# seung-lab/chunkflow

Measured on AMD Instinct MI355X. Metric: output_voxels_per_sec, higher is better.
Workload: dtype f32; 1 GPU; config2-512cube-rsunet-affinity; batch_size=12, engine=rsunet

## Files before the change

### chunkflow_amd/csrc/updown.hip

```cpp
#include <hip/hip_runtime.h>
#include <hip/hip_bf16.h>

#include "cfx_internal.h"

namespace {

typedef __hip_bfloat16 cfx_bf16;

template <typename T>
__device__ __forceinline__ float ldf(const T* p);
template <>
__device__ __forceinline__ float ldf<float>(const float* p) { return *p; }
template <>
__device__ __forceinline__ float ldf<cfx_bf16>(const cfx_bf16* p) {
    return __bfloat162float(*p);
}
__device__ __forceinline__ float cvf(float v) { return v; }
__device__ __forceinline__ float cvf(cfx_bf16 v) {
    return __bfloat162float(v);
}

template <typename T>
struct vec4;
template <>
struct vec4<float> {
    typedef float type __attribute__((ext_vector_type(4)));
    static __device__ __forceinline__ float get(type v, int i) {
        return v[i];
    }
};
template <>
struct vec4<cfx_bf16> {
    typedef unsigned short type __attribute__((ext_vector_type(4)));
    static __device__ __forceinline__ float get(type v, int i) {
        return __bfloat162float(
            __hip_bfloat16(__hip_bfloat16_raw{(unsigned short)v[i]}));
    }
};
template <typename T>
__device__ __forceinline__ void stf(T* p, float v);
template <>
__device__ __forceinline__ void stf<float>(float* p, float v) { *p = v; }
template <>
__device__ __forceinline__ void stf<cfx_bf16>(cfx_bf16* p, float v) {
    *p = __float2bfloat16(v);
}

template <typename T>
__device__ __forceinline__ void stage_rows(
    float* s_in, const T* in, const long long* row_off, int rows, int xn,
    int xvalid, int C, int CPAD, int tid, int nthreads) {
    const int total = rows * xn * C;
    for (int idx = tid; idx < total; idx += nthreads) {
        const int c = idx % C;
// ... 17 lines not shown
    float* s_in = smem + C * K * 4;
    const int CPAD = C | 1;
    const int tid = threadIdx.x;
    const int kslot = tid & 31;
    const int pslot = tid >> 5;

    for (int idx = tid; idx < C * K * 4; idx += 256) {
        const int q = idx & 3;
        const int k = (idx >> 2) % K;
        const int c = (idx >> 2) / K;
        s_w[(c * K + k) * 4 + q] = ldf(&wgt[(q * C + c) * K + k]);
    }

    const int nz = blockIdx.z;
    const int y = blockIdx.y;
    const int x0 = blockIdx.x * XI;
    const int xvalid = min(XI, W - x0);
    long long row_off[1] = {((((long long)nz * H) + y) * W + x0) * C};
    stage_rows(s_in, in, row_off, 1, XI, xvalid, C, CPAD, tid, 256);
    __syncthreads();

    const long long out_base =
        ((((long long)nz * 2 * H) + 2 * y) * 2 * W) * K;

    for (int k = kslot; k < K; k += 32) {
        const float bj = bias ? bias[k] : 0.f;
        float acc[PX][4];
#pragma unroll
        for (int p = 0; p < PX; ++p)
#pragma unroll
            for (int q = 0; q < 4; ++q) acc[p][q] = bj;
        for (int c = 0; c < C; ++c) {
            const float4 w4 =
                *reinterpret_cast<const float4*>(&s_w[(c * K + k) * 4]);
#pragma unroll
            for (int p = 0; p < PX; ++p) {
                const float v = s_in[(pslot + p * 8) * CPAD + c];
                acc[p][0] += v * w4.x;
                acc[p][1] += v * w4.y;
                acc[p][2] += v * w4.z;
                acc[p][3] += v * w4.w;
            }
        }
#pragma unroll
        for (int p = 0; p < PX; ++p) {
            const int xi = x0 + pslot + p * 8;
            if (xi >= W) continue;
            T* op = out + out_base + (long long)2 * xi * K + k;
            stf(op, acc[p][0]);
            stf(op + K, acc[p][1]);
            stf(op + (long long)2 * W * K, acc[p][2]);
            stf(op + (long long)2 * W * K + K, acc[p][3]);
        }
    }
}

template <typename T, int XO>
__global__ __launch_bounds__(256, 2) void k_downconv2(
    const T* __restrict__ in, const T* __restrict__ wgt,
    const float* __restrict__ bias, T* __restrict__ out, int N, int D,
    int H, int W, int C, int K) {
    constexpr int PX = XO / 8;
    extern __shared__ float smem[];
    float* s_w = smem;
    float* s_in = smem + C * K * 4;
    const int CPAD = C | 1;
    const int tid = threadIdx.x;
    const int kslot = tid & 31;
    const int pslot = tid >> 5;
    const int HO = H >> 1, WO = W >> 1;

    for (int idx = tid; idx < C * K * 4; idx += 256) {
        const int q = idx & 3;
        const int k = (idx >> 2) % K;
        const int c = (idx >> 2) / K;
        s_w[(c * K + k) * 4 + q] = ldf(&wgt[(q * C + c) * K + k]);
    }

    const int nz = blockIdx.z;
    const int y = blockIdx.y;
    const int x0 = blockIdx.x * XO;
    const int xvalid = min(2 * XO, W - 2 * x0);
    long long row_off[2] = {
        ((((long long)nz * H) + 2 * y) * W + 2 * x0) * C,
        ((((long long)nz * H) + 2 * y + 1) * W + 2 * x0) * C};
    stage_rows(s_in, in, row_off, 2, 2 * XO, xvalid, C, CPAD, tid, 256);
    __syncthreads();

    const long long out_row = (((long long)nz * HO) + y) * WO * K;

    for (int k = kslot; k < K; k += 32) {
        const float bj = bias ? bias[k] : 0.f;
        float acc[PX];
#pragma unroll
        for (int p = 0; p < PX; ++p) acc[p] = bj;
        for (int c = 0; c < C; ++c) {
            const float4 w4 =
                *reinterpret_cast<const float4*>(&s_w[(c * K + k) * 4]);
#pragma unroll
            for (int p = 0; p < PX; ++p) {
                const int xl = 2 * (pslot + p * 8);
                acc[p] += s_in[xl * CPAD + c] * w4.x;
                acc[p] += s_in[(xl + 1) * CPAD + c] * w4.y;
                acc[p] += s_in[(2 * XO + xl) * CPAD + c] * w4.z;
                acc[p] += s_in[(2 * XO + xl + 1) * CPAD + c] * w4.w;
            }
// ... 225 lines not shown
    const int q = tid - yl * (CO_S / 4);
    const int y = y0 + yl;
    const int gx = x0 + q * 4;
    if (y >= H || gx >= W) return;
    float o[4][3];
#pragma unroll
    for (int e = 0; e < 4; ++e)
#pragma unroll
        for (int k = 0; k < 3; ++k) o[e][k] = bias ? bias[k] : 0.f;
#pragma unroll
    for (int j = 0; j < 15; ++j) {
        const int dx = j / 3, k = j % 3;
        const float* pr = &s_p[(yl * 16 + j) * CO_PS + q * 4];
        const co_f32x4 lo = *reinterpret_cast<const co_f32x4*>(pr);
        const co_f32x4 hi = *reinterpret_cast<const co_f32x4*>(pr + 4);
        const float p8[8] = {lo[0], lo[1], lo[2], lo[3],
                             hi[0], hi[1], hi[2], hi[3]};
#pragma unroll
        for (int e = 0; e < 4; ++e) o[e][k] += p8[e + dx];
    }
    T* op = out + ((plane + y) * W + gx) * 3LL;
    if (vec_ok) {
        if (sizeof(T) == 2) {
            typedef unsigned co_u32x2 __attribute__((ext_vector_type(2)));
            unsigned short h[12];
#pragma unroll
            for (int i = 0; i < 12; ++i) h[i] = bf16_bits(o[i / 3][i % 3]);
#pragma unroll
            for (int i = 0; i < 3; ++i) {
                co_u32x2 u;
                u.x = h[4 * i] | ((unsigned)h[4 * i + 1] << 16);
                u.y = h[4 * i + 2] | ((unsigned)h[4 * i + 3] << 16);
                reinterpret_cast<co_u32x2*>(op)[i] = u;
            }
        } else {
#pragma unroll
            for (int i = 0; i < 3; ++i) {
                co_f32x4 f;
#pragma unroll
                for (int m = 0; m < 4; ++m)
                    f[m] = o[(4 * i + m) / 3][(4 * i + m) % 3];
                reinterpret_cast<co_f32x4*>(op)[i] = f;
            }
        }
    } else {
#pragma unroll
        for (int e = 0; e < 4; ++e)
            if (gx + e < W)
#pragma unroll
                for (int k = 0; k < 3; ++k) stf(&op[e * 3 + k], o[e][k]);
    }
}

}

extern "C" int cfx_conv155_out(cfx_ctx* ctx, const void* in,
                               const float* wfrag, const float* bias,
                               void* out, int N, int D, int H, int W,
                               int C, int K, int is_bf16) {
    if (C != 28 || K != 3) {
        g_err = "cfx_conv155_out: only C == 28, K == 3 instantiated";
        return -1;
    }
    if ((long long)N * D > 65535) {
        g_err = "cfx_conv155_out: N * D <= 65535 supported";
        return -1;
    }
    hipEvent_t e0;
    if (prof_begin(ctx, &e0)) return -1;
    dim3 grid((W + CO_S - 1) / CO_S, (H + CO_R - 1) / CO_R,
              (unsigned)(N * D));
    const int vec_ok = W % 4 == 0 && ((size_t)out & 15) == 0;
    if (is_bf16)
        hipLaunchKernelGGL((k_conv155_out_mfma<cfx_bf16>), grid, dim3(256),
                           0, ctx->stream, (const cfx_bf16*)in, wfrag, bias,
                           (cfx_bf16*)out, H, W, vec_ok);
    else
        hipLaunchKernelGGL((k_conv155_out_mfma<float>), grid, dim3(256), 0,
                           ctx->stream, (const float*)in, wfrag, bias,
                           (float*)out, H, W, vec_ok);
    CFX_CHECK(hipGetLastError());
    double flops = 2.0 * 25.0 * C * K * (double)N * D * H * W;
    if (prof_end(ctx, e0, CFX_K_CONV_STREAM, flops)) return -1;
    return 0;
}

extern "C" int cfx_conv155_c1(cfx_ctx* ctx, const void* in, const void* wgt,
                              const float* bias, void* out, int N, int D,
                              int H, int W, int K, int is_bf16) {
    if (K > 32) {
        g_err = "cfx_conv155_c1: K <= 32 supported";
        return -1;
    }
    constexpr int XI = 256;
    dim3 grid((W + XI - 1) / XI, H, (unsigned)(N * D));
    hipEvent_t e0;
    if (prof_begin(ctx, &e0)) return -1;
    if (is_bf16 && K == 28)
        hipLaunchKernelGGL((k_conv155_c1<cfx_bf16, XI, 28>), grid,
                           dim3(XI), 0, ctx->stream, (const cfx_bf16*)in,
                           (const cfx_bf16*)wgt, bias, (cfx_bf16*)out, N,
                           D, H, W, K);
    else if (is_bf16)
        hipLaunchKernelGGL((k_conv155_c1<cfx_bf16, XI, 0>), grid,
                           dim3(XI), 0, ctx->stream, (const cfx_bf16*)in,
                           (const cfx_bf16*)wgt, bias, (cfx_bf16*)out, N,
                           D, H, W, K);
    else if (K == 28)
        hipLaunchKernelGGL((k_conv155_c1<float, XI, 28>), grid, dim3(XI),
                           0, ctx->stream, (const float*)in,
                           (const float*)wgt, bias, (float*)out, N, D, H,
                           W, K);
    else
        hipLaunchKernelGGL((k_conv155_c1<float, XI, 0>), grid, dim3(XI),
                           0, ctx->stream, (const float*)in,
                           (const float*)wgt, bias, (float*)out, N, D, H,
                           W, K);
    CFX_CHECK(hipGetLastError());
    double flops = 2.0 * 25.0 * K * (double)N * D * H * W;
    if (prof_end(ctx, e0, CFX_K_CONV_STREAM, flops)) return -1;
    return 0;
}

extern "C" int cfx_upconv_2x2(cfx_ctx* ctx, const void* in, const void* wgt,
                              const float* bias, void* out, int N, int D,
                              int H, int W, int C, int K, int is_bf16) {
    if (K > 64 || C > 64) {
        g_err = "cfx_upconv_2x2: C, K <= 64 supported";
        return -1;
    }
    constexpr int XI = 64;
    dim3 grid((W + XI - 1) / XI, H, (unsigned)(N * D));
    const size_t shmem =
        ((size_t)C * K * 4 + (size_t)XI * (C | 1)) * sizeof(float);
    hipEvent_t e0;
    if (prof_begin(ctx, &e0)) return -1;
    if (is_bf16)
        hipLaunchKernelGGL((k_upconv2<cfx_bf16, XI>), grid, dim3(256),
                           shmem, ctx->stream, (const cfx_bf16*)in,
                           (const cfx_bf16*)wgt, bias, (cfx_bf16*)out, N, D,
                           H, W, C, K);
    else
        hipLaunchKernelGGL((k_upconv2<float, XI>), grid, dim3(256), shmem,
                           ctx->stream, (const float*)in, (const float*)wgt,
                           bias, (float*)out, N, D, H, W, C, K);
    CFX_CHECK(hipGetLastError());
    double flops = 2.0 * 4.0 * C * K * (double)N * D * H * W;
    if (prof_end(ctx, e0, CFX_K_CONV_STREAM, flops)) return -1;
    return 0;
}

extern "C" int cfx_downconv_2x2(cfx_ctx* ctx, const void* in,
                                const void* wgt, const float* bias,
                                void* out, int N, int D, int H, int W,
                                int C, int K, int is_bf16) {
    if (K > 64 || C > 64) {
        g_err = "cfx_downconv_2x2: C, K <= 64 supported";
        return -1;
    }
    if ((H | W) & 1) {
        g_err = "cfx_downconv_2x2: H, W must be even";
        return -1;
    }
    constexpr int XO = 64;
    dim3 grid((W / 2 + XO - 1) / XO, H / 2, (unsigned)(N * D));
    const size_t shmem =
        ((size_t)C * K * 4 + (size_t)2 * 2 * XO * (C | 1)) * sizeof(float);
    hipEvent_t e0;
    if (prof_begin(ctx, &e0)) return -1;
    if (is_bf16)
        hipLaunchKernelGGL((k_downconv2<cfx_bf16, XO>), grid, dim3(256),
                           shmem, ctx->stream, (const cfx_bf16*)in,
                           (const cfx_bf16*)wgt, bias, (cfx_bf16*)out, N, D,
                           H, W, C, K);
    else
        hipLaunchKernelGGL((k_downconv2<float, XO>), grid, dim3(256), shmem,
                           ctx->stream, (const float*)in, (const float*)wgt,
                           bias, (float*)out, N, D, H, W, C, K);
    CFX_CHECK(hipGetLastError());
    double flops = 2.0 * 4.0 * C * K * (double)N * D * (H / 2) * (W / 2);
    if (prof_end(ctx, e0, CFX_K_CONV_STREAM, flops)) return -1;
    return 0;
}
```

### chunkflow_amd/engines/pytorch.py

```python
import os

import torch

from .base import EngineBase
from ..model_loader import load_source


class PyTorchEngine(EngineBase):
    pre_masked = False

    def __init__(self, convnet_model, convnet_weight_path, **kw):
        super().__init__(convnet_model, convnet_weight_path, **kw)
        net_source = load_source(convnet_model)
        if hasattr(net_source, 'load_model'):
            self.model = net_source.load_model(convnet_weight_path)
        else:
            self.model = net_source.InstantiatedModel
            if convnet_weight_path is not None:
                chkpt = torch.load(convnet_weight_path,
                                   map_location='cpu')
                state_dict = chkpt.get('state_dict', chkpt) \
                    if isinstance(chkpt, dict) else chkpt
                self.model.load_state_dict(state_dict)
        self.model = self.model.to(self.device)
        self.model.eval()
        if self.dtype == 'bfloat16':
            self.model = self.model.to(torch.bfloat16)
        self.channels_last = (str(self.device).startswith('cuda') and
                              os.environ.get('CFX_CHANNELS_LAST', '1') != '0')
        if self.channels_last:
            self.model = self.model.to(memory_format=torch.channels_last_3d)
            if os.environ.get('CFX_FASTCONV', '1') != '0':
                idx = int(str(self.device).split(':')[-1])                     if ':' in str(self.device) else 0
                from ..fastconv import (accelerate_conv_in,
                                        accelerate_updown)
                bf = self.dtype == 'bfloat16'
                if bf:
                    from ..fastconv import maybe_accelerate_bf16
                    self.fastconv_count = maybe_accelerate_bf16(
                        self.model, idx)
                else:
                    from ..fastconv import maybe_accelerate
                    self.fastconv_count = maybe_accelerate(self.model, idx)
                self.fastconv_count += accelerate_updown(
                    self.model, idx, bf16=bf)
                self.fastconv_count += accelerate_conv_in(
                    self.model, idx, bf16=bf)
                from ..fastconv import accelerate_conv_out
                self.fastconv_count += accelerate_conv_out(
                    self.model, idx, bf16=bf)
        torch.backends.cudnn.benchmark = True
        self.pre_process = getattr(net_source, 'pre_process', None)
        self.post_process = getattr(net_source, 'post_process', None)

    @torch.no_grad()
    def __call__(self, batch):
        x = batch
        if self.pre_process is not None:
            x = self.pre_process(x)
        if self.dtype == 'bfloat16':
            x = x.to(torch.bfloat16)
        if self.channels_last:
            x = x.contiguous(memory_format=torch.channels_last_3d)
        out = self.model(x)
        if self.post_process is not None:
            out = self.post_process(out)
        if out.dtype != torch.float32:
            out = out.to(torch.float32)
        out = self._crop_output_patch(out)
        return out.contiguous()
```

### chunkflow_amd/fastconv.py

```python
import os

import torch
import torch.nn as nn

_CTX = {}


def get_cfx(device_index: int = 0):
    if device_index not in _CTX:
        from .hip import CfxContext
        ctx = CfxContext(device_index)
        ctx.adopt_torch_stream()
        _CTX[device_index] = ctx
    return _CTX[device_index]


ELIGIBLE_WIDTHS = (28, 36)
ZRING_WIDTHS = (28, 36)


def _eligible(m: nn.Module) -> bool:
    return (isinstance(m, nn.Conv3d)
            and m.kernel_size == (3, 3, 3)
            and m.stride == (1, 1, 1)
# ... 9 lines not shown
    def __init__(self, conv: nn.Conv3d, device_index: int = 0):
        super().__init__()
        self.C = conv.in_channels
        self.K = conv.out_channels
        self.device_index = device_index
        w = conv.weight.detach()
        wtap = w.permute(2, 3, 4, 1, 0).reshape(27, self.C, self.K)
        self.register_buffer('wtap', wtap.contiguous().float())
        if conv.bias is not None:
            self.register_buffer('bias', conv.bias.detach().float())
        else:
            self.bias = None

    def _run(self, x, residual=None, elu=False):
        x = x.contiguous(memory_format=torch.channels_last_3d)
        n, c, d, h, w = x.shape
        out = torch.empty((n, self.K, d, h, w), dtype=torch.float32,
                          device=x.device,
                          memory_format=torch.channels_last_3d)
        get_cfx(self.device_index).conv3_ndhwc(
            x.data_ptr(), self.wtap.data_ptr(),
            self.bias.data_ptr() if self.bias is not None else None,
            residual.data_ptr() if residual is not None else None,
            out.data_ptr(), n, d, h, w, self.C, self.K, do_elu=elu,
            zring=self.C in ZRING_WIDTHS)
        return out

    def forward(self, x):
        assert x.dtype == torch.float32, 'fastconv is the f32 path'
        return self._run(x)


class CfxResBlock(nn.Module):

    def __init__(self, block: nn.Module, device_index: int = 0):
        super().__init__()
        self.c1 = CfxConv3d(block.conv1, device_index)
        self.c2 = CfxConv3d(block.conv2, device_index)

    def forward(self, x):
        x = x.contiguous(memory_format=torch.channels_last_3d)
        h = self.c1._run(x, elu=True)
        return self.c2._run(h, residual=x, elu=True)


def _resblock_like(m: nn.Module) -> bool:
    return (hasattr(m, 'conv1') and hasattr(m, 'conv2')
            and isinstance(getattr(m, 'act', None), nn.ELU)
            and getattr(m.act, 'alpha', None) == 1.0
            and not isinstance(m, (CfxConv3d, CfxResBlock))
            and _eligible(m.conv1) and _eligible(m.conv2))


@torch.no_grad()
def _fusion_matches(block: nn.Module, fused: 'CfxResBlock') -> bool:
    C = fused.c1.C
    x = torch.randn(1, C, 4, 18, 22, device=fused.c1.wtap.device)         .contiguous(memory_format=torch.channels_last_3d)
    want = block.to(x.device)(x)
    got = fused(x)
    return bool(torch.allclose(got, want, rtol=1e-4, atol=1e-4))


def maybe_accelerate(model: nn.Module, device_index: int = 0) -> int:
    count = 0
    dev = f'cuda:{device_index}'
    fused_out = set()
    for parent in list(model.modules()):
        if id(parent) in fused_out:
            continue
        for name, child in list(parent.named_children()):
            if _resblock_like(child):
                fused = CfxResBlock(child, device_index).to(dev)
                if _fusion_matches(child, fused):
                    setattr(parent, name, fused)
                    fused_out.add(id(child))
                    count += 1
                    continue
                for cn in ('conv1', 'conv2'):
                    setattr(child, cn,
                            CfxConv3d(getattr(child, cn),
                                      device_index).to(dev))
                    count += 1
            elif _eligible(child):
                setattr(parent, name,
                        CfxConv3d(child, device_index).to(dev))
                count += 1
    return count


BF16_WIDTHS = tuple(
    int(w) for w in os.environ.get('CFX_BF16_WIDTHS', '28,36').split(',')
    if w)


class CfxConv3dBF16(nn.Module):

    def __init__(self, conv: nn.Conv3d, device_index: int = 0):
        super().__init__()
        self.C = conv.in_channels
        self.K = conv.out_channels
        self.device_index = device_index
        w = conv.weight.detach().float()
        if self.C <= 32:
            pack = torch.zeros(27, 32, 32)
        else:
            pack = torch.zeros(27, 64, 48)
        pack[:, :self.K, :self.C] = w.permute(2, 3, 4, 0, 1) \
            .reshape(27, self.K, self.C)
        self.register_buffer('wpack', pack.to(torch.bfloat16).contiguous())
        if conv.bias is not None:
            self.register_buffer('bias', conv.bias.detach().float())
        else:
            self.bias = None

    def _run(self, x, residual=None, elu=False):
        assert x.dtype == torch.bfloat16
        x = x.contiguous(memory_format=torch.channels_last_3d)
        n, c, d, h, w = x.shape
        out = torch.empty((n, self.K, d, h, w), dtype=torch.bfloat16,
                          device=x.device,
                          memory_format=torch.channels_last_3d)
        get_cfx(self.device_index).conv3_ndhwc_bf16(
            x.data_ptr(), self.wpack.data_ptr(),
            self.bias.data_ptr() if self.bias is not None else None,
            residual.data_ptr() if residual is not None else None,
            out.data_ptr(), n, d, h, w, self.C, self.K, do_elu=elu)
        return out

    def forward(self, x):
        return self._run(x)


class CfxResBlockBF16(nn.Module):
    def __init__(self, block: nn.Module, device_index: int = 0):
# ... 27 lines not shown

    @torch.no_grad()
    def matches(block, fused):
        x = torch.randn(1, fused.c1.C, 4, 18, 22, device=dev) \
            .to(torch.bfloat16) \
            .contiguous(memory_format=torch.channels_last_3d)
        want = block.to(dev)(x)
        got = fused(x)
        return bool(torch.allclose(got.float(), want.float(), rtol=0.05,
                                   atol=0.05))

    fused_out = set()
    for parent in list(model.modules()):
        if id(parent) in fused_out:
            continue
        for name, child in list(parent.named_children()):
            if rb(child):
                fused = CfxResBlockBF16(child, device_index).to(dev)
                if matches(child, fused):
                    setattr(parent, name, fused)
                    fused_out.add(id(child))
                    count += 1
                    continue
                for cn in ('conv1', 'conv2'):
                    setattr(child, cn,
                            CfxConv3dBF16(getattr(child, cn),
                                          device_index).to(dev))
                    count += 1
            elif elig(child):
                setattr(parent, name,
                        CfxConv3dBF16(child, device_index).to(dev))
                count += 1
    return count


class CfxUpConv3d(nn.Module):

    def __init__(self, conv: nn.ConvTranspose3d, device_index: int = 0,
                 bf16: bool = False):
        super().__init__()
        self.C = conv.in_channels
        self.K = conv.out_channels
        self.device_index = device_index
        self.bf16 = bf16
        w = conv.weight.detach().float()
        pack = w[:, :, 0].permute(2, 3, 0, 1).reshape(4, self.C, self.K)
        dt = torch.bfloat16 if bf16 else torch.float32
        self.register_buffer('wpack', pack.to(dt).contiguous())
        if conv.bias is not None:
            self.register_buffer('bias', conv.bias.detach().float())
        else:
            self.bias = None

    def forward(self, x):
        x = x.contiguous(memory_format=torch.channels_last_3d)
        n, c, d, h, w = x.shape
        dt = torch.bfloat16 if self.bf16 else torch.float32
        assert x.dtype == dt
        out = torch.empty((n, self.K, d, 2 * h, 2 * w), dtype=dt,
                          device=x.device,
                          memory_format=torch.channels_last_3d)
        get_cfx(self.device_index).upconv_2x2(
            x.data_ptr(), self.wpack.data_ptr(),
            self.bias.data_ptr() if self.bias is not None else None,
            out.data_ptr(), n, d, h, w, self.C, self.K, bf16=self.bf16)
        return out


class CfxDownConv3d(nn.Module):

    def __init__(self, conv: nn.Conv3d, device_index: int = 0,
                 bf16: bool = False):
        super().__init__()
        self.C = conv.in_channels
        self.K = conv.out_channels
        self.device_index = device_index
        self.bf16 = bf16
        w = conv.weight.detach().float()
        pack = w[:, :, 0].permute(2, 3, 1, 0).reshape(4, self.C, self.K)
        dt = torch.bfloat16 if bf16 else torch.float32
        self.register_buffer('wpack', pack.to(dt).contiguous())
        if conv.bias is not None:
            self.register_buffer('bias', conv.bias.detach().float())
        else:
            self.bias = None

    def forward(self, x):
        x = x.contiguous(memory_format=torch.channels_last_3d)
        n, c, d, h, w = x.shape
        dt = torch.bfloat16 if self.bf16 else torch.float32
        assert x.dtype == dt
        out = torch.empty((n, self.K, d, h // 2, w // 2), dtype=dt,
                          device=x.device,
                          memory_format=torch.channels_last_3d)
        get_cfx(self.device_index).downconv_2x2(
            x.data_ptr(), self.wpack.data_ptr(),
            self.bias.data_ptr() if self.bias is not None else None,
            out.data_ptr(), n, d, h, w, self.C, self.K, bf16=self.bf16)
        return out


UP_SURGERY_WIDTHS = (36, 48)


def _up_eligible(m) -> bool:
    return (isinstance(m, nn.ConvTranspose3d)
            and m.kernel_size == (1, 2, 2) and m.stride == (1, 2, 2)
            and m.padding == (0, 0, 0) and m.output_padding == (0, 0, 0)
            and m.dilation == (1, 1, 1) and m.groups == 1
            and m.in_channels in UP_SURGERY_WIDTHS
            and m.out_channels <= 64)


def _down_eligible(m) -> bool:
    return (isinstance(m, nn.Conv3d)
            and m.kernel_size == (1, 2, 2) and m.stride == (1, 2, 2)
            and m.padding == (0, 0, 0) and m.dilation == (1, 1, 1)
            and m.groups == 1
            and m.in_channels <= 64 and m.out_channels <= 64)


@torch.no_grad()
def _updown_matches(orig, repl, dev, bf16):
    x = torch.randn(1, repl.C, 3, 12, 16, device=dev)
    if bf16:
        x = x.to(torch.bfloat16)
    x = x.contiguous(memory_format=torch.channels_last_3d)
    want = orig.to(dev)(x).float()
    got = repl(x).float()
    tol = 0.05 if bf16 else 1e-4
    return bool(torch.allclose(got, want, rtol=tol, atol=tol))


def accelerate_updown(model: nn.Module, device_index: int = 0,
                      bf16: bool = False) -> int:
    count = 0
    dev = f'cuda:{device_index}'
    for parent in list(model.modules()):
        for name, child in list(parent.named_children()):
            repl = None
            if _up_eligible(child):
                repl = CfxUpConv3d(child, device_index, bf16=bf16).to(dev)
            if repl is not None and _updown_matches(child, repl, dev, bf16):
                setattr(parent, name, repl)
                count += 1
    return count


class CfxConvIn155(nn.Module):

    def __init__(self, conv: nn.Conv3d, device_index: int = 0,
                 bf16: bool = False):
        super().__init__()
        self.K = conv.out_channels
        self.device_index = device_index
        self.bf16 = bf16
        w = conv.weight.detach().float()
        dt = torch.bfloat16 if bf16 else torch.float32
        self.register_buffer('wpack',
                             w.reshape(self.K, 25).to(dt).contiguous())
        if conv.bias is not None:
            self.register_buffer('bias', conv.bias.detach().float())
        else:
            self.bias = None

    def forward(self, x):
        x = x.contiguous(memory_format=torch.channels_last_3d)
        n, c, d, h, w = x.shape
        assert c == 1
        dt = torch.bfloat16 if self.bf16 else torch.float32
        assert x.dtype == dt
        out = torch.empty((n, self.K, d, h, w), dtype=dt, device=x.device,
                          memory_format=torch.channels_last_3d)
        get_cfx(self.device_index).conv155_c1(
            x.data_ptr(), self.wpack.data_ptr(),
            self.bias.data_ptr() if self.bias is not None else None,
            out.data_ptr(), n, d, h, w, self.K, bf16=self.bf16)
        return out


def _conv155_eligible(m) -> bool:
    return (isinstance(m, nn.Conv3d) and m.kernel_size == (1, 5, 5)
            and m.stride == (1, 1, 1) and m.padding == (0, 2, 2)
            and m.dilation == (1, 1, 1) and m.groups == 1
            and m.in_channels == 1 and m.out_channels <= 32)


@torch.no_grad()
def _conv155_matches(orig, repl, dev, bf16):
    x = torch.randn(1, 1, 3, 14, 19, device=dev)
    if bf16:
        x = x.to(torch.bfloat16)
    x = x.contiguous(memory_format=torch.channels_last_3d)
    want = orig.to(dev)(x).float()
    got = repl(x).float()
    tol = 0.05 if bf16 else 1e-4
    return bool(torch.allclose(got, want, rtol=tol, atol=tol))


# ... 83 lines not shown
```

### chunkflow_amd/hip.py

```python
import ctypes
import os

import numpy as np

from .build import SO_PATH, build

SYMBOLS = [
    'cfx_init', 'cfx_destroy', 'cfx_last_error', 'cfx_version',
    'cfx_set_stream', 'cfx_sync', 'cfx_make_patch_mask',
    'cfx_normalize_intensity', 'cfx_cast_u8_f32_div', 'cfx_extract_patches',
    'cfx_blend_accumulate', 'cfx_blend_batch', 'cfx_build_chunk_mask',
    'cfx_reciprocal',
    'cfx_multiply_mask', 'cfx_multiply_mask_max', 'cfx_max',
    'cfx_crop_margin',
    'cfx_mask_using_last_channel', 'cfx_threshold', 'cfx_nonzero_u8',
    'cfx_connected_components', 'cfx_connected_components_labels',
    'cfx_label_run_starts', 'cfx_label_table_clear',
    'cfx_label_table_insert', 'cfx_label_count', 'cfx_label_mask',
    'cfx_hist_u8', 'cfx_lut_apply_u8',
    'cfx_downsample_avg_u8', 'cfx_downsample_avg_f32',
    'cfx_downsample_mode2', 'cfx_downsample_mode3',
    'cfx_conv3_ndhwc', 'cfx_conv3_ndhwc_w32',
    'cfx_conv3_ndhwc_zring', 'cfx_conv3_ndhwc_bf16',
    'cfx_upconv_2x2', 'cfx_downconv_2x2', 'cfx_conv155_c1',
    'cfx_conv155_out',
    'cfx_profile_enable', 'cfx_profile_reset',
    'cfx_profile_get',
]

KERNEL_IDS = {
    'blend': 0, 'extract': 1, 'normalize': 2, 'cast': 3, 'reciprocal': 4,
    'maskmul': 5, 'crop': 6, 'max': 7, 'myelin': 8, 'cc': 9, 'conv': 10,
    'conv_stream': 11, 'labels': 12,
}

_lib = None


class CfxError(RuntimeError):
    pass


def _i3(v):
    return (ctypes.c_int * 3)(*[int(x) for x in v])


def _i6(v):
    return (ctypes.c_int * 6)(*[int(x) for x in v])


def load_library(build_if_missing: bool = True):
    global _lib
    if _lib is not None:
        return _lib
    path = SO_PATH
    if not os.path.exists(path):
        if not build_if_missing:
            raise CfxError(f'HIP extension not built: {path}')
        path = build()
    lib = ctypes.CDLL(path)
    for sym in SYMBOLS:
        if not hasattr(lib, sym):
            raise CfxError(f'{path} is missing symbol {sym}')
    lib.cfx_init.restype = ctypes.c_void_p
    lib.cfx_init.argtypes = [ctypes.c_int]
    lib.cfx_last_error.restype = ctypes.c_char_p
    lib.cfx_destroy.argtypes = [ctypes.c_void_p]
    _lib = lib
    return lib


def extension_available() -> bool:
    try:
        load_library(build_if_missing=False)
        return True
    except Exception:
        return False

# ... 178 lines not shown
        self._chk(self.lib.cfx_label_table_clear(
            ctypes.c_void_p(self.ctx), ctypes.c_void_p(keys_ptr),
            ctypes.c_void_p(vals_ptr), ctypes.c_longlong(capacity)),
            'cfx_label_table_clear')

    def label_table_insert(self, ids_ptr, n_ids, value, keys_ptr, vals_ptr,
                           capacity):
        self._chk(self.lib.cfx_label_table_insert(
            ctypes.c_void_p(self.ctx), ctypes.c_void_p(ids_ptr),
            ctypes.c_longlong(n_ids), ctypes.c_uint(value),
            ctypes.c_void_p(keys_ptr), ctypes.c_void_p(vals_ptr),
            ctypes.c_longlong(capacity)), 'cfx_label_table_insert')

    def label_count(self, labels_ptr, elem_bytes, dims, keys_ptr, vals_ptr,
                    capacity):
        self._chk(self.lib.cfx_label_count(
            ctypes.c_void_p(self.ctx), ctypes.c_void_p(labels_ptr),
            ctypes.c_int(elem_bytes), _i3(dims), ctypes.c_void_p(keys_ptr),
            ctypes.c_void_p(vals_ptr), ctypes.c_longlong(capacity)),
            'cfx_label_count')

    def label_mask(self, in_ptr, out_ptr, elem_bytes, dims, keys_ptr,
                   vals_ptr, capacity, mode, threshold=0):
        self._chk(self.lib.cfx_label_mask(
            ctypes.c_void_p(self.ctx), ctypes.c_void_p(in_ptr),
            ctypes.c_void_p(out_ptr), ctypes.c_int(elem_bytes), _i3(dims),
            ctypes.c_void_p(keys_ptr), ctypes.c_void_p(vals_ptr),
            ctypes.c_longlong(capacity), ctypes.c_int(mode),
            ctypes.c_longlong(threshold)), 'cfx_label_mask')

    def conv3_ndhwc_bf16(self, in_ptr, wgt_ptr, bias_ptr, residual_ptr,
                         out_ptr, n, d, h, w, c, k, do_elu=False):
        self._chk(self.lib.cfx_conv3_ndhwc_bf16(
            ctypes.c_void_p(self.ctx), ctypes.c_void_p(in_ptr),
            ctypes.c_void_p(wgt_ptr),
            ctypes.c_void_p(bias_ptr) if bias_ptr else None,
            ctypes.c_void_p(residual_ptr) if residual_ptr else None,
            ctypes.c_void_p(out_ptr), ctypes.c_int(n), ctypes.c_int(d),
            ctypes.c_int(h), ctypes.c_int(w), ctypes.c_int(c),
            ctypes.c_int(k), ctypes.c_int(1 if do_elu else 0)),
            'cfx_conv3_ndhwc_bf16')

    def upconv_2x2(self, in_ptr, wgt_ptr, bias_ptr, out_ptr, n, d, h, w,
                   c, k, bf16=False):
        self._chk(self.lib.cfx_upconv_2x2(
            ctypes.c_void_p(self.ctx), ctypes.c_void_p(in_ptr),
            ctypes.c_void_p(wgt_ptr),
            ctypes.c_void_p(bias_ptr) if bias_ptr else None,
            ctypes.c_void_p(out_ptr), ctypes.c_int(n), ctypes.c_int(d),
            ctypes.c_int(h), ctypes.c_int(w), ctypes.c_int(c),
            ctypes.c_int(k), ctypes.c_int(1 if bf16 else 0)),
            'cfx_upconv_2x2')

    def downconv_2x2(self, in_ptr, wgt_ptr, bias_ptr, out_ptr, n, d, h, w,
                     c, k, bf16=False):
        self._chk(self.lib.cfx_downconv_2x2(
            ctypes.c_void_p(self.ctx), ctypes.c_void_p(in_ptr),
            ctypes.c_void_p(wgt_ptr),
            ctypes.c_void_p(bias_ptr) if bias_ptr else None,
            ctypes.c_void_p(out_ptr), ctypes.c_int(n), ctypes.c_int(d),
            ctypes.c_int(h), ctypes.c_int(w), ctypes.c_int(c),
            ctypes.c_int(k), ctypes.c_int(1 if bf16 else 0)),
            'cfx_downconv_2x2')

    def conv155_c1(self, in_ptr, wgt_ptr, bias_ptr, out_ptr, n, d, h, w,
                   k, bf16=False):
        self._chk(self.lib.cfx_conv155_c1(
            ctypes.c_void_p(self.ctx), ctypes.c_void_p(in_ptr),
            ctypes.c_void_p(wgt_ptr),
            ctypes.c_void_p(bias_ptr) if bias_ptr else None,
            ctypes.c_void_p(out_ptr), ctypes.c_int(n), ctypes.c_int(d),
            ctypes.c_int(h), ctypes.c_int(w), ctypes.c_int(k),
            ctypes.c_int(1 if bf16 else 0)), 'cfx_conv155_c1')

    def conv155_out(self, in_ptr, wgt_ptr, bias_ptr, out_ptr, n, d, h, w,
                    c, k, bf16=False):
        self._chk(self.lib.cfx_conv155_out(
            ctypes.c_void_p(self.ctx), ctypes.c_void_p(in_ptr),
            ctypes.c_void_p(wgt_ptr),
            ctypes.c_void_p(bias_ptr) if bias_ptr else None,
            ctypes.c_void_p(out_ptr), ctypes.c_int(n), ctypes.c_int(d),
            ctypes.c_int(h), ctypes.c_int(w), ctypes.c_int(c),
            ctypes.c_int(k), ctypes.c_int(1 if bf16 else 0)),
            'cfx_conv155_out')

    def hist_u8(self, in_ptr, n_per_sec, nsec, hist_ptr):
        self._chk(self.lib.cfx_hist_u8(
            ctypes.c_void_p(self.ctx), ctypes.c_void_p(in_ptr),
            ctypes.c_longlong(n_per_sec), ctypes.c_int(nsec),
            ctypes.c_void_p(hist_ptr)), 'cfx_hist_u8')

    def lut_apply_u8(self, buf_ptr, n_per_sec, nsec, lut_ptr):
        self._chk(self.lib.cfx_lut_apply_u8(
            ctypes.c_void_p(self.ctx), ctypes.c_void_p(buf_ptr),
            ctypes.c_longlong(n_per_sec), ctypes.c_int(nsec),
            ctypes.c_void_p(lut_ptr)), 'cfx_lut_apply_u8')

    def downsample_avg(self, in_ptr, out_ptr, channels, in_dims, factor,
                       is_f32=False):
        fn = (self.lib.cfx_downsample_avg_f32 if is_f32
              else self.lib.cfx_downsample_avg_u8)
        self._chk(fn(
            ctypes.c_void_p(self.ctx), ctypes.c_void_p(in_ptr),
            ctypes.c_void_p(out_ptr), ctypes.c_int(channels), _i3(in_dims),
            _i3(factor)), 'cfx_downsample_avg')

# ... 62 lines not shown
```

### include/chunkflow_amd.h

```cpp
#ifndef CHUNKFLOW_AMD_H
#define CHUNKFLOW_AMD_H

#ifdef __cplusplus
extern "C" {
#endif

typedef struct cfx_ctx cfx_ctx;

cfx_ctx* cfx_init(int device);
void     cfx_destroy(cfx_ctx* ctx);
const char* cfx_last_error(void);
int      cfx_version(void);
int cfx_set_stream(cfx_ctx* ctx, void* hip_stream);
int cfx_sync(cfx_ctx* ctx);

int cfx_make_patch_mask(const int patch_size[3], const int overlap[3],
                        float* out);

int cfx_normalize_intensity(cfx_ctx* ctx, const unsigned char* in, float* out,
                            long long n);
int cfx_cast_u8_f32_div(cfx_ctx* ctx, const unsigned char* in, float* out,
                        long long n, float divisor);
int cfx_extract_patches(cfx_ctx* ctx, const float* chunk, int channels,
                        const int chunk_dims[3], const int* starts_zyx,
// ... 34 lines not shown
                                    int elem_bytes, const int dims[3],
                                    int connectivity, unsigned int* labels,
                                    unsigned int* scratch,
                                    long long* n_components);

int cfx_label_run_starts(cfx_ctx* ctx, const void* labels, int elem_bytes,
                         const int dims[3], long long* n_runs);
int cfx_label_table_clear(cfx_ctx* ctx, unsigned long long* keys,
                          unsigned int* vals, long long capacity);
int cfx_label_table_insert(cfx_ctx* ctx, const unsigned long long* ids,
                           long long n_ids, unsigned int value,
                           unsigned long long* keys, unsigned int* vals,
                           long long capacity);
int cfx_label_count(cfx_ctx* ctx, const void* labels, int elem_bytes,
                    const int dims[3], unsigned long long* keys,
                    unsigned int* vals, long long capacity);
int cfx_label_mask(cfx_ctx* ctx, const void* in, void* out, int elem_bytes,
                   const int dims[3], const unsigned long long* keys,
                   const unsigned int* vals, long long capacity, int mode,
                   long long threshold);

int cfx_hist_u8(cfx_ctx* ctx, const unsigned char* in, long long n_per_sec,
                int nsec, unsigned int* hist);
int cfx_lut_apply_u8(cfx_ctx* ctx, unsigned char* buf, long long n_per_sec,
                     int nsec, const unsigned char* lut);

int cfx_downsample_avg_u8(cfx_ctx* ctx, const unsigned char* in,
                          unsigned char* out, int channels,
                          const int in_dims[3], const int factor[3]);
int cfx_downsample_avg_f32(cfx_ctx* ctx, const float* in, float* out,
                           int channels, const int in_dims[3],
                           const int factor[3]);
int cfx_downsample_mode2(cfx_ctx* ctx, const void* in, void* out,
                         int elem_bytes, const int in_dims[3],
                         int preserved_axis);
int cfx_downsample_mode3(cfx_ctx* ctx, const void* in, void* out,
                         int elem_bytes, const int in_dims[3]);

int cfx_conv3_ndhwc(cfx_ctx* ctx, const float* in, const float* wgt,
                    const float* bias, const float* residual, float* out,
                    int N, int D, int H, int W, int C, int K, int do_elu);
int cfx_conv3_ndhwc_zring(cfx_ctx* ctx, const float* in, const float* wgt,
                          const float* bias, const float* residual,
                          float* out, int N, int D, int H, int W, int C,
                          int K, int do_elu);
int cfx_conv3_ndhwc_bf16(cfx_ctx* ctx, const void* in, const void* wgt,
                         const float* bias, const void* residual,
                         void* out, int N, int D, int H, int W, int C,
                         int K, int do_elu);

int cfx_upconv_2x2(cfx_ctx* ctx, const void* in, const void* wgt,
                   const float* bias, void* out, int N, int D, int H,
                   int W, int C, int K, int is_bf16);
int cfx_downconv_2x2(cfx_ctx* ctx, const void* in, const void* wgt,
                     const float* bias, void* out, int N, int D, int H,
                     int W, int C, int K, int is_bf16);
int cfx_conv155_c1(cfx_ctx* ctx, const void* in, const void* wgt,
                   const float* bias, void* out, int N, int D, int H,
                   int W, int K, int is_bf16);
int cfx_conv155_out(cfx_ctx* ctx, const void* in, const float* wfrag,
                    const float* bias, void* out, int N, int D, int H,
                    int W, int C, int K, int is_bf16);
int cfx_conv3_ndhwc_w32(cfx_ctx* ctx, const float* in, const float* wgt,
                        const float* bias, const float* residual,
                        float* out, int N, int D, int H, int W, int C,
                        int K, int do_elu);

enum cfx_kernel_id {
    CFX_K_BLEND = 0,
    CFX_K_EXTRACT = 1,
    CFX_K_NORMALIZE = 2,
    CFX_K_CAST = 3,
    CFX_K_RECIPROCAL = 4,
    CFX_K_MASKMUL = 5,
    CFX_K_CROP = 6,
    CFX_K_MAX = 7,
    CFX_K_MYELIN = 8,
    CFX_K_CC = 9,
    CFX_K_CONV = 10,
    CFX_K_CONV_STREAM = 11,
    CFX_K_LABELS = 12,
    CFX_K_COUNT = 13
};
int cfx_profile_enable(cfx_ctx* ctx, int enable);
int cfx_profile_reset(cfx_ctx* ctx);
int cfx_profile_get(cfx_ctx* ctx, int kernel_id, unsigned long long* count,
                    double* total_ms, double* bytes);

#ifdef __cplusplus
}
#endif
#endif
```

Baseline: 105.3 million voxels/s.

## Add MFMA upconv with fused skip-add, FX fusion pass, and MIOpen resblock epilogue

```diff
diff --git a/chunkflow_amd/csrc/updown.hip b/chunkflow_amd/csrc/updown.hip
--- a/chunkflow_amd/csrc/updown.hip
+++ b/chunkflow_amd/csrc/updown.hip
@@ -1,5 +1,7 @@
 #include <hip/hip_runtime.h>
 #include <hip/hip_bf16.h>
+
+#include <algorithm>
 
 #include "cfx_internal.h"
 
@@ -123,6 +125,146 @@
             stf(op + (long long)2 * W * K, acc[p][2]);
             stf(op + (long long)2 * W * K + K, acc[p][3]);
         }
+    }
+}
+
+
+constexpr int UM_NW = 4;
+
+typedef float um_f32x4 __attribute__((ext_vector_type(4)));
+
+template <int NT, bool SKIP>
+__global__ __launch_bounds__(UM_NW * 64) void k_upconv2_mfma(
+    const float* __restrict__ in, const float* __restrict__ wgt,
+    const float* __restrict__ bias, const float* __restrict__ skip,
+    float* __restrict__ out, int W, int C, int xtiles, int ntiles) {
+    constexpr int K = 4 * NT;
+    constexpr int N4 = 4 * K;
+    constexpr int BS = N4 + 4;
+    constexpr int RUN4 = 2 * NT;
+    extern __shared__ __attribute__((aligned(16))) float um_smem[];
+    const int S = C >> 2;
+    const int tid = threadIdx.x;
+    const int lane = tid & 63;
+    const int wave = __builtin_amdgcn_readfirstlane(tid >> 6);
+    float* s_w = um_smem;
+    float* s_b = um_smem + C * N4 + wave * (16 * BS);
+
+    for (int idx = tid; idx < C * N4; idx += UM_NW * 64) {
+        const int l = idx & 63;
+        const int st = idx >> 6;
+        const int t = st % NT;
+        const int s = st / NT;
+        const int c = 4 * s + (l >> 4);
+        const int col = 16 * t + (l & 15);
+        const int q = col / K;
+        s_w[idx] = wgt[(q * C + c) * K + (col - q * K)];
+    }
+    __syncthreads();
+
+    const int ai = lane & 15;
+    const int akk = lane >> 4;
+    float bj[NT];
+#pragma unroll
+    for (int t = 0; t < NT; ++t)
+        bj[t] = bias ? bias[(16 * t + ai) % K] : 0.f;
+
+    auto piece = [&](int it, int& py, int& i, int& j4) {
+        const int f = it * 64 + lane;
+        py = f >= 16 * RUN4;
+        const int rem = f - py * (16 * RUN4);
+        i = rem / RUN4;
+        j4 = rem - i * RUN4;
+    };
+    auto a_loads = [&](int tile, float (&a)[16]) {
+        const int xt = tile % xtiles;
+        const long long row = tile / xtiles;
+        const int x0 = xt * 16;
+        const int ilast = min(16, W - x0) - 1;
+        const float* ip = in + (row * W + x0) * C;
+        const unsigned ao = min(ai, ilast) * C + akk;
+#pragma unroll
+        for (int s = 0; s < 16; ++s) a[s] = ip[ao + 4u * min(s, S - 1)];
+    };
+    auto skip_loads = [&](int tile, um_f32x4 (&sv)[NT]) {
+        const int xt = tile % xtiles;
+        const long long row = tile / xtiles;
+        const int x0 = xt * 16;
+        const int ilast = min(16, W - x0) - 1;
+        const float* sp = skip + (2 * row * 2 * W + 2 * x0) * K;
+#pragma unroll
+        for (int it = 0; it < NT; ++it) {
+            int py, i, j4;
+            piece(it, py, i, j4);
+            const unsigned so =
+                py * (2 * W * K) + min(i, ilast) * (2 * K) + 4 * j4;
+            sv[it] = *reinterpret_cast<const um_f32x4*>(sp + so);
+        }
+    };
+
+    auto do_tile = [&](int tile, int next, const float (&a)[16],
+                       float (&a2)[16]) {
+        um_f32x4 sv[NT];
+        if (SKIP) skip_loads(tile, sv);
+        a_loads(next, a2);
+        __builtin_amdgcn_sched_barrier(0);
+        um_f32x4 acc[NT];
+#pragma unroll
+        for (int t = 0; t < NT; ++t)
+            acc[t] = um_f32x4{bj[t], bj[t], bj[t], bj[t]};
+#pragma unroll
+        for (int s = 0; s < 16; ++s) {
+            if (s >= S) break;
+#pragma unroll
+            for (int t = 0; t < NT; ++t)
+                acc[t] = __builtin_amdgcn_mfma_f32_16x16x4f32(
+                    a[s], s_w[(s * NT + t) * 64 + lane], acc[t], 0, 0, 0);
+        }
+#pragma unroll
+        for (int t = 0; t < NT; ++t)
+#pragma unroll
+            for (int r = 0; r < 4; ++r)
+                s_b[(akk * 4 + r) * BS + 16 * t + ai] = acc[t][r];
+        __builtin_amdgcn_wave_barrier();
+
+        const int xt = tile % xtiles;
+        const long long row = tile / xtiles;
+        const int x0 = xt * 16;
+        const int nvalid = min(16, W - x0);
+        float* op = out + (2 * row * 2 * W + 2 * x0) * K;
+        um_f32x4 v[NT];
+#pragma unroll
+        for (int it = 0; it < NT; ++it) {
+            int py, i, j4;
+            piece(it, py, i, j4);
+            v[it] = *reinterpret_cast<const um_f32x4*>(
+                &s_b[i * BS + py * (2 * K) + 4 * j4]);
+            if (SKIP) v[it] += sv[it];
+        }
+        __builtin_amdgcn_sched_barrier(0);
+#pragma unroll
+        for (int it = 0; it < NT; ++it) {
+            int py, i, j4;
+            piece(it, py, i, j4);
+            const unsigned oo = py * (2 * W * K) + i * (2 * K) + 4 * j4;
+            if (nvalid == 16 || i < nvalid)
+                *reinterpret_cast<um_f32x4*>(op + oo) = v[it];
+        }
+        __builtin_amdgcn_wave_barrier();
+    };
+
+    const int stride = gridDim.x * UM_NW;
+    int tile = blockIdx.x * UM_NW + wave;
+    if (tile >= ntiles) return;
+    float a0[16], a1[16];
+    a_loads(tile, a0);
+    while (true) {
+        do_tile(tile, min(tile + stride, ntiles - 1), a0, a1);
+        tile += stride;
+        if (tile >= ntiles) break;
+        do_tile(tile, min(tile + stride, ntiles - 1), a1, a0);
+        tile += stride;
+        if (tile >= ntiles) break;
     }
 }
 
@@ -454,6 +596,42 @@
     }
 }
 
+__device__ __forceinline__ float bre_act(float v, int do_elu) {
+    if (do_elu) {
+        const float e = expm1f(v > 0.f ? 0.f : v);
+        v = v > 0.f ? v : e;
+    }
+    return v;
+}
+
+template <bool VEC>
+__global__ __launch_bounds__(256) void k_bias_res_elu(
+    float* __restrict__ y, const float* __restrict__ bias,
+    const float* __restrict__ res, long long total, int K, int do_elu) {
+    const long long step = (long long)gridDim.x * 256;
+    long long i = (long long)blockIdx.x * 256 + threadIdx.x;
+    if (VEC) {
+        const long long n4 = total >> 2;
+        const int K4 = K >> 2;
+        for (; i < n4; i += step) {
+            const int k4 = (int)(i % K4);
+            um_f32x4 v = reinterpret_cast<const um_f32x4*>(y)[i];
+            if (bias) v += reinterpret_cast<const um_f32x4*>(bias)[k4];
+            if (res) v += reinterpret_cast<const um_f32x4*>(res)[i];
+#pragma unroll
+            for (int e = 0; e < 4; ++e) v[e] = bre_act(v[e], do_elu);
+            reinterpret_cast<um_f32x4*>(y)[i] = v;
+        }
+    } else {
+        for (; i < total; i += step) {
+            float v = y[i];
+            if (bias) v += bias[(int)(i % K)];
+            if (res) v += res[i];
+            y[i] = bre_act(v, do_elu);
+        }
+    }
+}
+
 }
 
 extern "C" int cfx_conv155_out(cfx_ctx* ctx, const void* in,
@@ -524,12 +702,107 @@
     return 0;
 }
 
+namespace {
+
+size_t um_shmem(int C, int K) {
+    return ((size_t)C * 4 * K + (size_t)UM_NW * 16 * (4 * K + 4)) *
+           sizeof(float);
+}
+
+bool um_eligible(const void* in, const void* skip, const void* out, int N,
+                 int D, int H, int W, int C, int K) {
+    return C % 4 == 0 && K % 4 == 0 && C >= 4 && C <= 64 && K >= 4 &&
+           K <= 48 && (((size_t)in | (size_t)skip | (size_t)out) & 15) == 0 &&
+           (long long)N * D * H * ((W + 15) / 16) < (1LL << 31);
+}
+
+template <int NT, bool SKIP>
+int um_launch_nt(cfx_ctx* ctx, const float* in, const float* wgt,
+                 const float* bias, const float* skip, float* out, int W,
+                 int C, int xtiles, int ntiles) {
+    const size_t shmem = um_shmem(C, 4 * NT);
+    if (shmem > 64 * 1024)
+        CFX_CHECK(hipFuncSetAttribute(
+            reinterpret_cast<const void*>(&k_upconv2_mfma<NT, SKIP>),
+            hipFuncAttributeMaxDynamicSharedMemorySize, (int)shmem));
+    int cus = 0;
+    CFX_CHECK(hipDeviceGetAttribute(
+        &cus, hipDeviceAttributeMultiprocessorCount, ctx->device));
+    const int per_cu = (int)std::min<size_t>(8, (160 * 1024) / shmem);
+    const int grid =
+        std::min((ntiles + UM_NW - 1) / UM_NW, std::max(1, cus * per_cu));
+    hipLaunchKernelGGL((k_upconv2_mfma<NT, SKIP>), dim3(grid),
+                       dim3(UM_NW * 64), shmem, ctx->stream, in, wgt, bias,
+                       skip, out, W, C, xtiles, ntiles);
+    CFX_CHECK(hipGetLastError());
+    return 0;
+}
+
+template <bool SKIP>
+int um_launch(cfx_ctx* ctx, const float* in, const float* wgt,
+              const float* bias, const float* skip, float* out, int N,
+              int D, int H, int W, int C, int K) {
+    const int xtiles = (W + 15) / 16;
+    const int ntiles = N * D * H * xtiles;
+    if (ntiles == 0) return 0;
+    switch (K / 4) {
+#define UM_CASE(NT)                                                         \
+    case NT:                                                                \
+        return um_launch_nt<NT, SKIP>(ctx, in, wgt, bias, skip, out, W, C,  \
+                                      xtiles, ntiles);
+        UM_CASE(1) UM_CASE(2) UM_CASE(3) UM_CASE(4) UM_CASE(5) UM_CASE(6)
+        UM_CASE(7) UM_CASE(8) UM_CASE(9) UM_CASE(10) UM_CASE(11)
+        UM_CASE(12)
+#undef UM_CASE
+    }
+    g_err = "upconv mfma: K not instantiated";
+    return -1;
+}
+
+}
+
+extern "C" int cfx_upconv_2x2_add(cfx_ctx* ctx, const void* in,
+                                  const void* wgt, const float* bias,
+                                  const void* skip, void* out, int N, int D,
+                                  int H, int W, int C, int K, int is_bf16) {
+    if (!skip)
+        return cfx_upconv_2x2(ctx, in, wgt, bias, out, N, D, H, W, C, K,
+                              is_bf16);
+    if (is_bf16) {
+        g_err = "cfx_upconv_2x2_add: skip is f32 only";
+        return -1;
+    }
+    if (!um_eligible(in, skip, out, N, D, H, W, C, K)) {
+        g_err = "cfx_upconv_2x2_add: skip needs C % 4 == 0, K % 4 == 0, "
+                "C <= 64, K <= 48 and 16-byte aligned tensors";
+        return -1;
+    }
+    hipEvent_t e0;
+    if (prof_begin(ctx, &e0)) return -1;
+    if (um_launch<true>(ctx, (const float*)in, (const float*)wgt, bias,
+                        (const float*)skip, (float*)out, N, D, H, W, C, K))
+        return -1;
+    double flops = 2.0 * 4.0 * C * K * (double)N * D * H * W;
+    if (prof_end(ctx, e0, CFX_K_CONV_STREAM, flops)) return -1;
+    return 0;
+}
+
 extern "C" int cfx_upconv_2x2(cfx_ctx* ctx, const void* in, const void* wgt,
                               const float* bias, void* out, int N, int D,
                               int H, int W, int C, int K, int is_bf16) {
     if (K > 64 || C > 64) {
         g_err = "cfx_upconv_2x2: C, K <= 64 supported";
         return -1;
+    }
+    if (!is_bf16 && um_eligible(in, nullptr, out, N, D, H, W, C, K)) {
+        hipEvent_t e0;
+        if (prof_begin(ctx, &e0)) return -1;
+        if (um_launch<false>(ctx, (const float*)in, (const float*)wgt, bias,
+                             nullptr, (float*)out, N, D, H, W, C, K))
+            return -1;
+        double flops = 2.0 * 4.0 * C * K * (double)N * D * H * W;
+        if (prof_end(ctx, e0, CFX_K_CONV_STREAM, flops)) return -1;
+        return 0;
     }
     constexpr int XI = 64;
     dim3 grid((W + XI - 1) / XI, H, (unsigned)(N * D));
@@ -584,3 +857,27 @@
     if (prof_end(ctx, e0, CFX_K_CONV_STREAM, flops)) return -1;
     return 0;
 }
+
+extern "C" int cfx_bias_res_elu(cfx_ctx* ctx, float* y, const float* bias,
+                                const float* res, long long nvox, int K,
+                                int do_elu) {
+    if (nvox < 0 || K < 1) {
+        g_err = "cfx_bias_res_elu: nvox >= 0, K >= 1";
+        return -1;
+    }
+    const long long total = nvox * K;
+    if (total == 0) return 0;
+    const bool vec =
+        K % 4 == 0 &&
+        (((size_t)y | (size_t)bias | (size_t)res) & 15) == 0;
+    const long long items = vec ? total / 4 : total;
+    const int grid = (int)std::min<long long>((items + 255) / 256, 256 * 16);
+    if (vec)
+        hipLaunchKernelGGL((k_bias_res_elu<true>), dim3(grid), dim3(256), 0,
+                           ctx->stream, y, bias, res, total, K, do_elu);
+    else
+        hipLaunchKernelGGL((k_bias_res_elu<false>), dim3(grid), dim3(256), 0,
+                           ctx->stream, y, bias, res, total, K, do_elu);
+    CFX_CHECK(hipGetLastError());
+    return 0;
+}
diff --git a/chunkflow_amd/engines/pytorch.py b/chunkflow_amd/engines/pytorch.py
--- a/chunkflow_amd/engines/pytorch.py
+++ b/chunkflow_amd/engines/pytorch.py
@@ -49,6 +49,11 @@
                 from ..fastconv import accelerate_conv_out
                 self.fastconv_count += accelerate_conv_out(
                     self.model, idx, bf16=bf)
+                self.upskip_count = 0
+                if not bf:
+                    from ..fastconv import accelerate_up_skip
+                    self.model, self.upskip_count = accelerate_up_skip(
+                        self.model, idx, self.num_input_channels)
         torch.backends.cudnn.benchmark = True
         self.pre_process = getattr(net_source, 'pre_process', None)
         self.post_process = getattr(net_source, 'post_process', None)
diff --git a/chunkflow_amd/fastconv.py b/chunkflow_amd/fastconv.py
--- a/chunkflow_amd/fastconv.py
+++ b/chunkflow_amd/fastconv.py
@@ -85,10 +85,64 @@
             and _eligible(m.conv1) and _eligible(m.conv2))
 
 
+def _conv333(m: nn.Module) -> bool:
+    return (isinstance(m, nn.Conv3d)
+            and m.kernel_size == (3, 3, 3)
+            and m.stride == (1, 1, 1)
+            and m.padding == (1, 1, 1)
+            and m.dilation == (1, 1, 1)
+            and m.groups == 1
+            and m.in_channels == m.out_channels)
+
+
+class CfxMiopenResBlock(nn.Module):
+
+    def __init__(self, block: nn.Module, device_index: int = 0):
+        super().__init__()
+        self.C = block.conv1.in_channels
+        self.device_index = device_index
+        for i, conv in ((1, block.conv1), (2, block.conv2)):
+            self.register_buffer(f'w{i}', conv.weight.detach())
+            self.register_buffer(
+                f'b{i}', conv.bias.detach().float().contiguous()
+                if conv.bias is not None else None)
+
+    def _conv(self, x, w, b, res):
+        y = torch.nn.functional.conv3d(x, w, None, padding=1)
+        y = y.contiguous(memory_format=torch.channels_last_3d)
+        n, k, d, h, wd = y.shape
+        get_cfx(self.device_index).bias_res_elu(
+            y.data_ptr(), b.data_ptr() if b is not None else None,
+            res.data_ptr() if res is not None else None,
+            n * d * h * wd, k, do_elu=True)
+        return y
+
+    def forward(self, x):
+        assert x.dtype == torch.float32, 'fastconv is the f32 path'
+        x = x.contiguous(memory_format=torch.channels_last_3d)
+        h = self._conv(x, self.w1, self.b1, None)
+        return self._conv(h, self.w2, self.b2, x)
+
+
+def _miopen_resblock_like(m: nn.Module) -> bool:
+    return (hasattr(m, 'conv1') and hasattr(m, 'conv2')
+            and isinstance(getattr(m, 'act', None), nn.ELU)
+            and getattr(m.act, 'alpha', None) == 1.0
+            and not isinstance(m, (CfxConv3d, CfxResBlock,
+                                   CfxMiopenResBlock))
+            and _conv333(m.conv1) and _conv333(m.conv2)
+            and m.conv1.in_channels == m.conv2.in_channels
+            and not _eligible(m.conv1) and not _eligible(m.conv2))
+
+
 @torch.no_grad()
-def _fusion_matches(block: nn.Module, fused: 'CfxResBlock') -> bool:
-    C = fused.c1.C
-    x = torch.randn(1, C, 4, 18, 22, device=fused.c1.wtap.device)         .contiguous(memory_format=torch.channels_last_3d)
+def _fusion_matches(block: nn.Module, fused: nn.Module) -> bool:
+    if isinstance(fused, CfxMiopenResBlock):
+        C, dev = fused.C, fused.w1.device
+    else:
+        C, dev = fused.c1.C, fused.c1.wtap.device
+    x = torch.randn(1, C, 4, 18, 22, device=dev) \
+        .contiguous(memory_format=torch.channels_last_3d)
     want = block.to(x.device)(x)
     got = fused(x)
     return bool(torch.allclose(got, want, rtol=1e-4, atol=1e-4))
@@ -113,6 +167,12 @@
                     setattr(child, cn,
                             CfxConv3d(getattr(child, cn),
                                       device_index).to(dev))
+                    count += 1
+            elif _miopen_resblock_like(child):
+                fused = CfxMiopenResBlock(child, device_index).to(dev)
+                if _fusion_matches(child, fused):
+                    setattr(parent, name, fused)
+                    fused_out.add(id(child))
                     count += 1
             elif _eligible(child):
                 setattr(parent, name,
@@ -246,7 +306,18 @@
         else:
             self.bias = None
 
-    def forward(self, x):
+    def _fusable(self, skip, out_shape) -> bool:
+        return (not self.bf16 and torch.is_tensor(skip)
+                and skip.dtype == torch.float32
+                and skip.device == self.wpack.device
+                and tuple(skip.shape) == tuple(out_shape)
+                and skip.is_contiguous(
+                    memory_format=torch.channels_last_3d)
+                and skip.data_ptr() % 16 == 0
+                and self.C % 4 == 0 and self.K % 4 == 0
+                and self.C <= 64 and self.K <= 48)
+
+    def forward(self, x, skip=None):
         x = x.contiguous(memory_format=torch.channels_last_3d)
         n, c, d, h, w = x.shape
         dt = torch.bfloat16 if self.bf16 else torch.float32
@@ -254,10 +325,15 @@
         out = torch.empty((n, self.K, d, 2 * h, 2 * w), dtype=dt,
                           device=x.device,
                           memory_format=torch.channels_last_3d)
-        get_cfx(self.device_index).upconv_2x2(
+        fuse = (skip is not None and self._fusable(skip, out.shape)
+                and x.data_ptr() % 16 == 0 and out.data_ptr() % 16 == 0)
+        get_cfx(self.device_index).upconv_2x2_add(
             x.data_ptr(), self.wpack.data_ptr(),
             self.bias.data_ptr() if self.bias is not None else None,
+            skip.data_ptr() if fuse else None,
             out.data_ptr(), n, d, h, w, self.C, self.K, bf16=self.bf16)
+        if skip is not None and not fuse:
+            return out + skip
         return out
 
 
@@ -295,14 +371,16 @@
 
 
 UP_SURGERY_WIDTHS = (36, 48)
-
-
-def _up_eligible(m) -> bool:
+UP_SURGERY_WIDTHS_F32 = (36, 48, 64)
+
+
+def _up_eligible(m, bf16: bool = False) -> bool:
+    widths = UP_SURGERY_WIDTHS if bf16 else UP_SURGERY_WIDTHS_F32
     return (isinstance(m, nn.ConvTranspose3d)
             and m.kernel_size == (1, 2, 2) and m.stride == (1, 2, 2)
             and m.padding == (0, 0, 0) and m.output_padding == (0, 0, 0)
             and m.dilation == (1, 1, 1) and m.groups == 1
-            and m.in_channels in UP_SURGERY_WIDTHS
+            and m.in_channels in widths
             and m.out_channels <= 64)
 
 
@@ -333,12 +411,86 @@
     for parent in list(model.modules()):
         for name, child in list(parent.named_children()):
             repl = None
-            if _up_eligible(child):
+            if _up_eligible(child, bf16):
                 repl = CfxUpConv3d(child, device_index, bf16=bf16).to(dev)
             if repl is not None and _updown_matches(child, repl, dev, bf16):
                 setattr(parent, name, repl)
                 count += 1
     return count
+
+
+def fuse_up_skip_adds(model: nn.Module, is_up=None):
+    import operator
+
+    import torch.fx as fx
+
+    if is_up is None:
+        def is_up(m):
+            return isinstance(m, CfxUpConv3d)
+
+    class _Tracer(fx.Tracer):
+        def is_leaf_module(self, m, qualname):
+            return not isinstance(m, (nn.ModuleList, nn.ModuleDict,
+                                      nn.Sequential))
+
+    try:
+        graph = _Tracer().trace(model)
+    except Exception:
+        return model, 0
+    mods = dict(model.named_modules())
+
+    def up_call(n):
+        return (isinstance(n, fx.Node) and n.op == 'call_module'
+                and is_up(mods.get(n.target)) and len(n.args) == 1
+                and not n.kwargs and len(n.users) == 1)
+
+    count = 0
+    for node in list(graph.nodes):
+        is_add = (node.op == 'call_function'
+                  and node.target in (operator.add, torch.add)) or \
+                 (node.op == 'call_method' and node.target == 'add')
+        if not is_add or len(node.args) != 2 or node.kwargs:
+            continue
+        a, b = node.args
+        if up_call(a) and isinstance(b, fx.Node) and b is not a:
+            up, other = a, b
+        elif up_call(b) and isinstance(a, fx.Node) and a is not b:
+            up, other = b, a
+        else:
+            continue
+        order = {n: i for i, n in enumerate(graph.nodes)}
+        if order[other] > order[up]:
+            continue
+        up.args = (up.args[0], other)
+        node.replace_all_uses_with(up)
+        graph.erase_node(node)
+        count += 1
+    if count == 0:
+        return model, 0
+    try:
+        graph.lint()
+        return fx.GraphModule(model, graph), count
+    except Exception:
+        return model, 0
+
+
+@torch.no_grad()
+def accelerate_up_skip(model: nn.Module, device_index: int = 0,
+                       in_channels: int = 1):
+    dev = f'cuda:{device_index}'
+    try:
+        fused, count = fuse_up_skip_adds(model)
+        if count == 0:
+            return model, 0
+        for shape in ((2, 16, 24), (3, 32, 16)):
+            x = torch.randn(1, in_channels, *shape, device=dev).contiguous(
+                memory_format=torch.channels_last_3d)
+            if not torch.allclose(fused(x), model(x), rtol=1e-4,
+                                  atol=1e-4):
+                return model, 0
+        return fused, count
+    except Exception:
+        return model, 0
 
 
 class CfxConvIn155(nn.Module):
diff --git a/chunkflow_amd/hip.py b/chunkflow_amd/hip.py
--- a/chunkflow_amd/hip.py
+++ b/chunkflow_amd/hip.py
@@ -22,8 +22,8 @@
     'cfx_downsample_mode2', 'cfx_downsample_mode3',
     'cfx_conv3_ndhwc', 'cfx_conv3_ndhwc_w32',
     'cfx_conv3_ndhwc_zring', 'cfx_conv3_ndhwc_bf16',
-    'cfx_upconv_2x2', 'cfx_downconv_2x2', 'cfx_conv155_c1',
-    'cfx_conv155_out',
+    'cfx_upconv_2x2', 'cfx_upconv_2x2_add', 'cfx_downconv_2x2',
+    'cfx_conv155_c1', 'cfx_conv155_out', 'cfx_bias_res_elu',
     'cfx_profile_enable', 'cfx_profile_reset',
     'cfx_profile_get',
 ]
@@ -308,6 +308,26 @@
             ctypes.c_int(k), ctypes.c_int(1 if bf16 else 0)),
             'cfx_upconv_2x2')
 
+    def upconv_2x2_add(self, in_ptr, wgt_ptr, bias_ptr, skip_ptr, out_ptr,
+                       n, d, h, w, c, k, bf16=False):
+        self._chk(self.lib.cfx_upconv_2x2_add(
+            ctypes.c_void_p(self.ctx), ctypes.c_void_p(in_ptr),
+            ctypes.c_void_p(wgt_ptr),
+            ctypes.c_void_p(bias_ptr) if bias_ptr else None,
+            ctypes.c_void_p(skip_ptr) if skip_ptr else None,
+            ctypes.c_void_p(out_ptr), ctypes.c_int(n), ctypes.c_int(d),
+            ctypes.c_int(h), ctypes.c_int(w), ctypes.c_int(c),
+            ctypes.c_int(k), ctypes.c_int(1 if bf16 else 0)),
+            'cfx_upconv_2x2_add')
+
+    def bias_res_elu(self, y_ptr, bias_ptr, res_ptr, nvox, k, do_elu=True):
+        self._chk(self.lib.cfx_bias_res_elu(
+            ctypes.c_void_p(self.ctx), ctypes.c_void_p(y_ptr),
+            ctypes.c_void_p(bias_ptr) if bias_ptr else None,
+            ctypes.c_void_p(res_ptr) if res_ptr else None,
+            ctypes.c_longlong(nvox), ctypes.c_int(k),
+            ctypes.c_int(1 if do_elu else 0)), 'cfx_bias_res_elu')
+
     def downconv_2x2(self, in_ptr, wgt_ptr, bias_ptr, out_ptr, n, d, h, w,
                      c, k, bf16=False):
         self._chk(self.lib.cfx_downconv_2x2(
diff --git a/include/chunkflow_amd.h b/include/chunkflow_amd.h
--- a/include/chunkflow_amd.h
+++ b/include/chunkflow_amd.h
@@ -110,6 +110,12 @@
 int cfx_upconv_2x2(cfx_ctx* ctx, const void* in, const void* wgt,
                    const float* bias, void* out, int N, int D, int H,
                    int W, int C, int K, int is_bf16);
+int cfx_upconv_2x2_add(cfx_ctx* ctx, const void* in, const void* wgt,
+                       const float* bias, const void* skip, void* out,
+                       int N, int D, int H, int W, int C, int K,
+                       int is_bf16);
+int cfx_bias_res_elu(cfx_ctx* ctx, float* y, const float* bias,
+                     const float* res, long long nvox, int K, int do_elu);
 int cfx_downconv_2x2(cfx_ctx* ctx, const void* in, const void* wgt,
                      const float* bias, void* out, int N, int D, int H,
                      int W, int C, int K, int is_bf16);
```

Result: faster. 110.4 million voxels/s, median of 6 (+4.9%).
